# ed-fish/data-efficient-video-transformers

Hardware: AMD Instinct MI355X
Metric: clips/sec fwd+bwd, B=8 T=32 3x224x224 bf16 (higher is better)
Workload: dtype bf16; 1 GPU; ViViT metric shape (SURVEY 8 'M'; BASELINE configs[2]/[3] transformer): B=8/GPU, T=32, 3x224x224, patch 16, d=512, ...; global_batch=8, parallelism=dp1

## Files before the change

### data-efficient-video-transformers_amd/csrc/attention.hip

```cpp
#include "common.h"
#include <cstdlib>

namespace {

__device__ __forceinline__ void wave_lds_sync() {
  asm volatile("s_waitcnt lgkmcnt(0)" ::: "memory");
  __builtin_amdgcn_wave_barrier();
}

constexpr float kLog2e = 1.4426950408889634f;
constexpr float kLn2 = 0.6931471805599453f;

struct AttnParams {
  const void *q, *k, *v, *o, *d_o;
  void *out, *dq, *dk, *dv;
  float* lse;
  float* delta;
  int B, H, Lq, Lk, dh;
  int64_t q_sb, q_sh, q_sl, k_sb, k_sh, k_sl, v_sb, v_sh, v_sl, o_sb, o_sh, o_sl;
  float scale;
  int Lkp;
  int Lqp;
  int patch_off;
  uint32_t drop_thr;
// ... 963 lines not shown
__global__ __launch_bounds__(1024) void attn_bwd_dkv_mfma_kernel(const AttnParams p) {
  extern __shared__ __attribute__((aligned(16))) char smem[];
  using V8 = typename Elem16<E>::v8;
  const int lane = threadIdx.x & 63, wid = threadIdx.x >> 6, W = blockDim.x >> 6;
  const int g = lane >> 4, li = lane & 15;
  const int b = blockIdx.x / p.H, h = blockIdx.x % p.H;
  const E* qb = (const E*)p.q + b * p.q_sb + h * p.q_sh;
  const E* kb = (const E*)p.k + b * p.k_sb + h * p.k_sh;
  const E* vb = (const E*)p.v + b * p.v_sb + h * p.v_sh;
  const E* gb = (const E*)p.d_o + b * p.o_sb + h * p.o_sh;
  E* dkb = (E*)p.dk + b * p.k_sb + h * p.k_sh;
  E* dvb = (E*)p.dv + b * p.v_sb + h * p.v_sh;
  const float* lse = p.lse + ((int64_t)b * p.H + h) * p.Lq;
  const float* delta = p.delta + ((int64_t)b * p.H + h) * p.Lq;
  char* qs = smem;
  char* gs = smem + p.Lqp * kRowBytes;
  float* l2s = reinterpret_cast<float*>(smem + 2 * p.Lqp * kRowBytes);
  float* dls = l2s + p.Lqp;
  const int nkt = (p.Lk + 15) >> 4, nqp = NQP ? NQP : p.Lqp >> 5;
  auto load_rows = [&](int kt, V8* kf, V8* vf) {
    const int kj = kt * 16 + li;
    const int krow = kj < p.Lk ? kj : p.Lk - 1;
#pragma unroll
    for (int kk = 0; kk < 2; ++kk) {
      kf[kk] = *reinterpret_cast<const V8*>(kb + (int64_t)krow * p.k_sl + kk * 32 + g * 8);
      vf[kk] = *reinterpret_cast<const V8*>(vb + (int64_t)krow * p.v_sl + kk * 32 + g * 8);
    }
  };
  V8 kf[2], vf[2];
  load_rows(wid, kf, vf);
  const int sr = (int)threadIdx.x < p.Lq ? (int)threadIdx.x : p.Lq - 1;
  const float lse0 = lse[sr], dl0 = delta[sr];
  stage_images<E>(qs, qb, p.q_sl, gs, gb, p.o_sl, p.Lq, p.Lqp);
  if ((int)threadIdx.x < p.Lqp) {
    l2s[threadIdx.x] = (int)threadIdx.x < p.Lq ? -lse0 * kLog2e : 0.f;
    dls[threadIdx.x] = (int)threadIdx.x < p.Lq ? -dl0 : 0.f;
  }
  for (int r = threadIdx.x + blockDim.x; r < p.Lqp; r += blockDim.x) {
    l2s[r] = r < p.Lq ? -lse[r] * kLog2e : 0.f;
    dls[r] = r < p.Lq ? -delta[r] : 0.f;
  }
  __syncthreads();

  const float c2 = p.scale * kLog2e;
  char* patch = p.patch_off >= 0 ? smem + p.patch_off + wid * 2048 : nullptr;
  for (int kt = wid; kt < nkt; kt += W) {
    asm volatile("" ::: "memory");
    f32x4 dk[4], dv[4];
#pragma unroll
    for (int dt = 0; dt < 4; ++dt) {
      dk[dt] = f32x4{0.f, 0.f, 0.f, 0.f};
      dv[dt] = f32x4{0.f, 0.f, 0.f, 0.f};
    }
    const f32x2 c2v = {c2, c2};
    auto step = [&](int qp) {
      f32x4 s[2], dp[2];
#pragma unroll
      for (int tt = 0; tt < 2; ++tt) {
        s[tt] = f32x4{0.f, 0.f, 0.f, 0.f};
        dp[tt] = f32x4{0.f, 0.f, 0.f, 0.f};
#pragma unroll
        for (int kk = 0; kk < 2; ++kk) {
          s[tt] = Elem16<E>::mma(img_row_frag<E>(qs, (2 * qp + tt) * 16, kk, g, li), kf[kk], s[tt]);
          dp[tt] = Elem16<E>::mma(img_row_frag<E>(gs, (2 * qp + tt) * 16, kk, g, li), vf[kk], dp[tt]);
        }
      }
#pragma unroll
      for (int tt = 0; tt < 2; ++tt) {
        const int q0 = (2 * qp + tt) * 16 + 4 * g;
        const f32x4 l2 = *reinterpret_cast<const f32x4*>(l2s + q0);
        const f32x4 dl = *reinterpret_cast<const f32x4*>(dls + q0);
#pragma unroll
        for (int r = 0; r < 4; r += 2) {
          const f32x2 x = __builtin_elementwise_fma(f32x2{s[tt][r], s[tt][r + 1]}, c2v, f32x2{l2[r], l2[r + 1]});
          const f32x2 d = f32x2{dp[tt][r], dp[tt][r + 1]} + f32x2{dl[r], dl[r + 1]};
          const f32x2 pr = {__builtin_amdgcn_exp2f(x[0]), __builtin_amdgcn_exp2f(x[1])};
          const f32x2 ds = pr * d;
          s[tt][r] = pr[0];
          s[tt][r + 1] = pr[1];
          dp[tt][r] = ds[0];
          dp[tt][r + 1] = ds[1];
        }
      }
      const V8 pf = pack_pair<E>(s[0], s[1]);
      const V8 dsf = pack_pair<E>(dp[0], dp[1]);
#pragma unroll
      for (int dt = 0; dt < 4; ++dt) {
        dv[dt] = Elem16<E>::mma(img_tr_frag<E>(gs, 2 * qp, 2 * qp + 1, dt * 16, g, li), pf, dv[dt]);
        dk[dt] = Elem16<E>::mma(img_tr_frag<E>(qs, 2 * qp, 2 * qp + 1, dt * 16, g, li), dsf, dk[dt]);
      }
    };
    if constexpr (NQP > 0) {
#pragma unroll
      for (int qp = 0; qp < NQP; ++qp) step(qp);
    } else {
      for (int qp = 0; qp < nqp; ++qp) step(qp);
    }
    if (kt + W < nkt) load_rows(kt + W, kf, vf);
    store_tile<E>(patch, dkb, p.k_sl, kt * 16, p.Lk, dk, p.scale, lane);
    store_tile<E>(patch, dvb, p.v_sl, kt * 16, p.Lk, dv, 1.0f, lane);
  }
}

constexpr int kStripRow = 80;

template <typename E>
__device__ __forceinline__ typename Elem16<E>::v8 strip_tr_frag(const char* strip, int ta, int tb, int col0, int g, int li) {
  const int qq = li >> 2, pp = li & 3;
  typename Elem16<E>::v4 half[2];
#pragma unroll
  for (int hf = 0; hf < 2; ++hf) {
    const int r = 16 * (hf ? tb : ta) + 4 * g + qq;
    half[hf] = Elem16<E>::tr_read(strip + r * kStripRow + col0 * 2 + 8 * pp);
  }
  return __builtin_shufflevector(half[0], half[1], 0, 1, 2, 3, 4, 5, 6, 7);
}

template <typename E, int NCH>
__device__ __forceinline__ void stage_bwd_operands(char* qs, const E* q, int64_t q_sl, char* gs, const E* g, const E* o, int64_t o_sl,
                                                   char* ks, const E* k, int64_t k_sl, int Lq, int Lk, int rows_pad, float* dls) {
  using V8 = typename Elem16<E>::v8;
  const int total = rows_pad * 8, nt = blockDim.x;
  V8 vq[NCH], vg[NCH], vo[NCH], vk[NCH];
#pragma unroll
  for (int u = 0; u < NCH; ++u) {
    const int idx = min((int)threadIdx.x + u * nt, total - 1);
    const int r = idx >> 3, c = idx & 7;
    const int rq = r < Lq ? r : 0, rk = r < Lk ? r : 0;
    vq[u] = *reinterpret_cast<const V8*>(q + (int64_t)rq * q_sl + c * 8);
    vg[u] = *reinterpret_cast<const V8*>(g + (int64_t)rq * o_sl + c * 8);
    vo[u] = *reinterpret_cast<const V8*>(o + (int64_t)rq * o_sl + c * 8);
    vk[u] = *reinterpret_cast<const V8*>(k + (int64_t)rk * k_sl + c * 8);
  }
  __builtin_amdgcn_sched_barrier(0);
  const V8 zero = {0, 0, 0, 0, 0, 0, 0, 0};
#pragma unroll
  for (int u = 0; u < NCH; ++u) {
    const int idx = min((int)threadIdx.x + u * nt, total - 1);
    const int r = idx >> 3, off = img_off(r, idx & 7);
    const bool lq = r < Lq, lk = r < Lk;
    *reinterpret_cast<V8*>(qs + off) = lq ? vq[u] : zero;
    *reinterpret_cast<V8*>(gs + off) = lq ? vg[u] : zero;
    *reinterpret_cast<V8*>(ks + off) = lk ? vk[u] : zero;
    float d = 0.f;
#pragma unroll
    for (int j = 0; j < 8; ++j) d = fmaf((float)vg[u][j], (float)vo[u][j], d);
    d += __shfl_xor(d, 1, 64);
    d += __shfl_xor(d, 2, 64);
    d += __shfl_xor(d, 4, 64);
    if ((idx & 7) == 0) dls[r] = lq ? -d : 0.f;
  }
}

template <typename E, int NP>
__global__ __launch_bounds__(512) void attn_bwd_fused_kernel(const AttnParams p) {
  extern __shared__ __attribute__((aligned(16))) char smem[];
  using V8 = typename Elem16<E>::v8;
  using V4 = typename Elem16<E>::v4;
  constexpr int LP = 32 * NP;
  const int lane = threadIdx.x & 63;
  const int wid = __builtin_amdgcn_readfirstlane(threadIdx.x >> 6);
  const int W = blockDim.x >> 6, WC = W - 1;
  const int g = lane >> 4, li = lane & 15;
  const int b = blockIdx.x / p.H, h = blockIdx.x % p.H;
  const E* qb = (const E*)p.q + b * p.q_sb + h * p.q_sh;
  const E* kb = (const E*)p.k + b * p.k_sb + h * p.k_sh;
  const E* vb = (const E*)p.v + b * p.v_sb + h * p.v_sh;
  const E* ob = (const E*)p.o + b * p.o_sb + h * p.o_sh;
  const E* gb = (const E*)p.d_o + b * p.o_sb + h * p.o_sh;
  E* dqb = (E*)p.dq + b * p.q_sb + h * p.q_sh;
  E* dkb = (E*)p.dk + b * p.k_sb + h * p.k_sh;
  E* dvb = (E*)p.dv + b * p.v_sb + h * p.v_sh;
  const float* lse = p.lse + ((int64_t)b * p.H + h) * p.Lq;
  char* qs = smem;
  char* gs = qs + LP * kRowBytes;
  char* ks = gs + LP * kRowBytes;
  char* strip0 = ks + LP * kRowBytes;
  float* l2s = reinterpret_cast<float*>(strip0 + 2 * LP * kStripRow);
  float* dls = l2s + LP;
  char* patch = reinterpret_cast<char*>(dls + LP) + wid * 2048;

  V8 kf[2][2], vf[2][2];
  if (wid < WC) {
#pragma unroll
    for (int j = 0; j < 2; ++j) {
      const int kj = (2 * wid + j) * 16 + li;
      const int krow = kj < p.Lk ? kj : p.Lk - 1;
#pragma unroll
      for (int kk = 0; kk < 2; ++kk) {
        kf[j][kk] = *reinterpret_cast<const V8*>(kb + (int64_t)krow * p.k_sl + kk * 32 + g * 8);
        vf[j][kk] = *reinterpret_cast<const V8*>(vb + (int64_t)krow * p.v_sl + kk * 32 + g * 8);
      }
    }
  }
  {
    const int r = threadIdx.x;
    const float l = lse[r < p.Lq ? r : 0];
    stage_bwd_operands<E, 4>(qs, qb, p.q_sl, gs, gb, ob, p.o_sl, ks, kb, p.k_sl, p.Lq, p.Lk, LP, dls);
    if (r < LP) l2s[r] = r < p.Lq ? -l * kLog2e : 0.f;
  }
  __syncthreads();
  const float c2 = p.scale * kLog2e;
  if (wid < WC) {
    f32x4 dk[2][4], dv[2][4];
#pragma unroll
    for (int j = 0; j < 2; ++j)
#pragma unroll
      for (int dt = 0; dt < 4; ++dt) {
        dk[j][dt] = f32x4{0.f, 0.f, 0.f, 0.f};
        dv[j][dt] = f32x4{0.f, 0.f, 0.f, 0.f};
      }
    const f32x2 c2v = {c2, c2};
    const bool kvalid[2] = {(2 * wid) * 16 + li < p.Lk, (2 * wid + 1) * 16 + li < p.Lk};
    char* myrow[2] = {strip0 + ((2 * wid) * 16 + li) * kStripRow + g * 8, strip0 + ((2 * wid + 1) * 16 + li) * kStripRow + g * 8};
#pragma unroll
    for (int qp = 0; qp < NP; ++qp) {
      asm volatile("" ::: "memory");
      V8 qfr[2][2], gfr[2][2];
#pragma unroll
      for (int tt = 0; tt < 2; ++tt)
#pragma unroll
        for (int kk = 0; kk < 2; ++kk) {
          qfr[tt][kk] = img_row_frag<E>(qs, (2 * qp + tt) * 16, kk, g, li);
          gfr[tt][kk] = img_row_frag<E>(gs, (2 * qp + tt) * 16, kk, g, li);
        }
      f32x4 l2[2], dl[2];
#pragma unroll
      for (int tt = 0; tt < 2; ++tt) {
        l2[tt] = *reinterpret_cast<const f32x4*>(l2s + (2 * qp + tt) * 16 + 4 * g);
        dl[tt] = *reinterpret_cast<const f32x4*>(dls + (2 * qp + tt) * 16 + 4 * g);
      }
      V8 pf[2], dsf[2];
#pragma unroll
      for (int j = 0; j < 2; ++j) {
        f32x4 s[2], dp[2];
#pragma unroll
        for (int tt = 0; tt < 2; ++tt) {
          s[tt] = f32x4{0.f, 0.f, 0.f, 0.f};
          dp[tt] = f32x4{0.f, 0.f, 0.f, 0.f};
#pragma unroll
          for (int kk = 0; kk < 2; ++kk) {
            s[tt] = Elem16<E>::mma(qfr[tt][kk], kf[j][kk], s[tt]);
            dp[tt] = Elem16<E>::mma(gfr[tt][kk], vf[j][kk], dp[tt]);
          }
        }
#pragma unroll
        for (int tt = 0; tt < 2; ++tt)
#pragma unroll
          for (int r = 0; r < 4; r += 2) {
            const f32x2 x = __builtin_elementwise_fma(f32x2{s[tt][r], s[tt][r + 1]}, c2v, f32x2{l2[tt][r], l2[tt][r + 1]});
            const f32x2 d = f32x2{dp[tt][r], dp[tt][r + 1]} + f32x2{dl[tt][r], dl[tt][r + 1]};
            f32x2 pr = {__builtin_amdgcn_exp2f(x[0]), __builtin_amdgcn_exp2f(x[1])};
            if (!kvalid[j]) pr = f32x2{0.f, 0.f};
            const f32x2 ds = pr * d;
            s[tt][r] = pr[0];
            s[tt][r + 1] = pr[1];
            dp[tt][r] = ds[0];
            dp[tt][r + 1] = ds[1];
          }
        pf[j] = pack_pair<E>(s[0], s[1]);
        dsf[j] = pack_pair<E>(dp[0], dp[1]);
      }
#pragma unroll
      for (int j = 0; j < 2; ++j) {
        char* row = myrow[j] + (qp & 1) * (LP * kStripRow);
        *reinterpret_cast<V4*>(row) = __builtin_shufflevector(dsf[j], dsf[j], 0, 1, 2, 3);
        *reinterpret_cast<V4*>(row + 32) = __builtin_shufflevector(dsf[j], dsf[j], 4, 5, 6, 7);
      }
#pragma unroll
      for (int dt = 0; dt < 4; ++dt) {
        const V8 gt = img_tr_frag<E>(gs, 2 * qp, 2 * qp + 1, dt * 16, g, li);
        const V8 qt = img_tr_frag<E>(qs, 2 * qp, 2 * qp + 1, dt * 16, g, li);
#pragma unroll
        for (int j = 0; j < 2; ++j) {
          dv[j][dt] = Elem16<E>::mma(gt, pf[j], dv[j][dt]);
          dk[j][dt] = Elem16<E>::mma(qt, dsf[j], dk[j][dt]);
        }
      }
      __syncthreads();
    }
#pragma unroll
    for (int j = 0; j < 2; ++j) {
      const int k0 = (2 * wid + j) * 16;
      if (k0 < p.Lk) {
        store_tile<E>(patch, dkb, p.k_sl, k0, p.Lk, dk[j], p.scale, lane);
        store_tile<E>(patch, dvb, p.v_sl, k0, p.Lk, dv[j], 1.0f, lane);
      }
    }
  } else {
    V8 ka[NP][4];
#pragma unroll
    for (int kp = 0; kp < NP; ++kp)
#pragma unroll
      for (int dt = 0; dt < 4; ++dt) ka[kp][dt] = img_tr_frag<E>(ks, 2 * kp, 2 * kp + 1, dt * 16, g, li);
#pragma unroll 1
    for (int qp = 0; qp < NP; ++qp) {
      __syncthreads();
      const char* strip = strip0 + (qp & 1) * (LP * kStripRow);
      V8 bq[NP][2];
#pragma unroll
      for (int kp = 0; kp < NP; ++kp) {
        bq[kp][0] = strip_tr_frag<E>(strip, 2 * kp, 2 * kp + 1, 0, g, li);
        bq[kp][1] = strip_tr_frag<E>(strip, 2 * kp, 2 * kp + 1, 16, g, li);
      }
      f32x4 acc[2][4];
#pragma unroll
      for (int tt = 0; tt < 2; ++tt)
#pragma unroll
        for (int dt = 0; dt < 4; ++dt) acc[tt][dt] = f32x4{0.f, 0.f, 0.f, 0.f};
#pragma unroll
      for (int kp = 0; kp < NP; ++kp)
#pragma unroll
        for (int dt = 0; dt < 4; ++dt) {
          acc[0][dt] = Elem16<E>::mma(ka[kp][dt], bq[kp][0], acc[0][dt]);
          acc[1][dt] = Elem16<E>::mma(ka[kp][dt], bq[kp][1], acc[1][dt]);
        }
#pragma unroll
      for (int tt = 0; tt < 2; ++tt)
        if ((2 * qp + tt) * 16 < p.Lq) store_tile<E>(nullptr, dqb, p.q_sl, (2 * qp + tt) * 16, p.Lq, acc[tt], p.scale, lane);
    }
  }
}

constexpr int kMaxLds = 160 * 1024;

int fill_params(const dvt_attn_desc* d, AttnParams& p, bool bwd, const char* name) {
  DVT_REQUIRE(d, "%s: null descriptor", name);
  DVT_REQUIRE(d->q && d->k && d->v && d->o && d->lse, "%s: null q/k/v/o/lse", name);
  DVT_REQUIRE(d->B >= 0 && d->H > 0 && d->Lq > 0 && d->Lk > 0 && d->dh > 0, "%s: bad sizes", name);
  DVT_REQUIRE(d->B * d->H < (1ll << 31) && d->Lq < (1 << 24) && d->Lk < (1 << 24), "%s: sizes too large", name);
  if (bwd) DVT_REQUIRE(d->d_o && d->dq && d->dk && d->dv, "%s: null gradient pointer", name);
  p.q = d->q; p.k = d->k; p.v = d->v; p.o = d->o; p.out = d->o; p.d_o = d->d_o;
  p.dq = d->dq; p.dk = d->dk; p.dv = d->dv; p.lse = d->lse; p.delta = nullptr;
  p.B = (int)d->B; p.H = (int)d->H; p.Lq = (int)d->Lq; p.Lk = (int)d->Lk; p.dh = (int)d->dh;
  p.q_sb = d->q_sb; p.q_sh = d->q_sh; p.q_sl = d->q_sl;
  p.k_sb = d->k_sb; p.k_sh = d->k_sh; p.k_sl = d->k_sl;
  p.v_sb = d->v_sb; p.v_sh = d->v_sh; p.v_sl = d->v_sl;
  p.o_sb = d->o_sb; p.o_sh = d->o_sh; p.o_sl = d->o_sl;
  p.scale = d->scale;
  DVT_REQUIRE(d->dropout_p >= 0.f && d->dropout_p < 1.f, "%s: dropout_p must be in [0, 1)", name);
  DVT_REQUIRE(d->dropout_p == 0.f || d->rng_state, "%s: dropout needs rng_state", name);
  p.drop_thr = 0u; p.drop_scale = 1.f; p.rng = d->rng_state; p.rng_off = d->rng_offset;
  if (d->dropout_p > 0.f) {
    const double th = (double)d->dropout_p * 4294967296.0;
    p.drop_thr = th >= 4294967295.0 ? 0xFFFFFFFFu : (uint32_t)(th + 0.5);
    if (p.drop_thr == 0u) p.drop_thr = 1u;
    p.drop_scale = 1.0f / (1.0f - d->dropout_p);
  }
  p.Lkp = (p.Lk + 31) & ~31;
  p.Lqp = (p.Lq + 31) & ~31;
  p.patch_off = -1;

  return DVT_OK;
}

bool strides_vec_ok(const dvt_attn_desc* d) {
  const int64_t s[] = {d->q_sb, d->q_sh, d->q_sl, d->k_sb, d->k_sh, d->k_sl,
                       d->v_sb, d->v_sh, d->v_sl, d->o_sb, d->o_sh, d->o_sl};
  for (int64_t x : s)
    if (x % 8) return false;
  return true;
}

bool mfma_fwd_ok(const dvt_attn_desc* d, const AttnParams& p) {
  return d->dropout_p == 0.f && d->scale > 0.f && dvt_is_16bit(d->dtype) && d->dh == DH && strides_vec_ok(d) && dvt_aligned16(d->q) &&
         dvt_aligned16(d->k) && dvt_aligned16(d->v) && dvt_aligned16(d->o) &&
         2 * p.Lkp * kRowBytes <= kMaxLds;
}

bool q1_ok(const dvt_attn_desc* d, const AttnParams& p) {
  return p.Lq == 1 && d->dropout_p == 0.f && dvt_is_16bit(d->dtype) && d->dh == DH && strides_vec_ok(d) &&
         dvt_aligned16(d->q) && dvt_aligned16(d->k) && dvt_aligned16(d->v) && dvt_aligned16(d->o) &&
         (size_t)4 * p.Lkp * sizeof(float) <= (size_t)kMaxLds;
}

bool mfma_bwd_ok(const dvt_attn_desc* d, const AttnParams& p) {
  return mfma_fwd_ok(d, p) && dvt_aligned16(d->d_o) && dvt_aligned16(d->dq) && dvt_aligned16(d->dk) &&
         dvt_aligned16(d->dv) && 2 * p.Lqp * kRowBytes + 2 * p.Lqp * 4 <= kMaxLds;
}

bool fused_bwd_ok(const AttnParams& p) { return p.Lqp == p.Lkp && p.Lkp <= 224; }
size_t fused_bwd_lds(int NP, int waves) {
  const size_t LP = 32 * (size_t)NP;
  return 3 * LP * kRowBytes + 2 * LP * kStripRow + 2 * LP * sizeof(float) + (size_t)waves * 2048;
}

int pick_waves(int tiles, size_t lds_bytes, int cap = 16) {
  int maxw = lds_bytes > 80 * 1024 ? 16 : 8;
  if (maxw > cap) maxw = cap;
  const int rounds = (tiles + maxw - 1) / maxw;
  int w = (tiles + rounds - 1) / rounds;
  return w < 1 ? 1 : w;
}

size_t with_patches(size_t lds, int waves, AttnParams& p) {
  const size_t tot = lds + (size_t)waves * 2048;
  const bool ok = lds <= 80 * 1024 ? 2 * tot <= (size_t)kMaxLds : tot <= (size_t)kMaxLds;
  p.patch_off = ok ? (int)lds : -1;
  return ok ? tot : lds;
}

template <typename K>
int set_lds(K kernel, size_t bytes) {
  if (bytes > 64 * 1024) {
    const hipError_t e = hipFuncSetAttribute((const void*)kernel, hipFuncAttributeMaxDynamicSharedMemorySize, (int)bytes);
    if (e != hipSuccess) return dvt_fail_hip(e, "hipFuncSetAttribute(MaxDynamicSharedMemorySize)");
  }
  return 0;
}

int resolve_fwd(const dvt_attn_desc* d, AttnParams& p, dvt_attn_plan_info& r) {
  r = dvt_attn_plan_info{};
  r.patch = r.patch2 = -1;
  int rc = fill_params(d, p, false, "dvt_attention_fwd");
  if (rc) return rc;
  if (p.B == 0) return DVT_OK;
  if (q1_ok(d, p)) {
    r.family = DVT_ATTN_F_Q1; r.waves = 4; r.lds = (int64_t)4 * p.Lkp * sizeof(float);
    return DVT_OK;
  }
  if (mfma_fwd_ok(d, p)) {
    const size_t lds_img = (size_t)2 * p.Lkp * kRowBytes;
    const int nkp = p.Lkp >> 5;
    r.waves = pick_waves((p.Lq + 15) / 16, lds_img, nkp > 7 && nkp <= 11 ? 12 : 16);
    r.lds = (int64_t)with_patches(lds_img, r.waves, p);
    r.patch = p.patch_off >= 0;
    r.family = nkp <= 11 ? DVT_ATTN_F_RES : DVT_ATTN_F_ONLINE;
    r.count = nkp <= 11 ? nkp : 0;
    return DVT_OK;
  }
  const int nt_s = p.Lq * p.dh >= 4096 ? 512 : 256;
  const size_t lds_s = ((size_t)(p.Lq + 2 * p.Lk) * small_dhp(p.dh) +
                        (size_t)small_parts(p.Lq, p.Lk, nt_s) * p.Lq * small_lp(p.Lk)) * sizeof(float);
  if (d->dtype != DVT_F32 && d->dtype != DVT_BF16 && d->dtype != DVT_F16)
    DVT_UNSUPPORTED("dvt_attention_fwd: dtype %d not supported", d->dtype);
  if (p.Lq <= kSmallL && p.Lk <= kSmallL && p.dh <= kSmallDh && lds_s <= (size_t)kMaxLds) {
    r.family = DVT_ATTN_F_SMALL; r.waves = nt_s / 64; r.lds = (int64_t)lds_s;
    return DVT_OK;
  }
  const size_t lds = (size_t)4 * (p.dh + p.Lk) * sizeof(float);
  if (lds > (size_t)kMaxLds) DVT_UNSUPPORTED("dvt_attention_fwd: Lk = %d, dh = %d exceed the LDS budget", p.Lk, p.dh);
  r.family = DVT_ATTN_F_GENERIC; r.waves = 4; r.lds = (int64_t)lds;
  return DVT_OK;
}

int resolve_bwd(const dvt_attn_desc* d, AttnParams& p, AttnParams& pq, AttnParams& pkv, dvt_attn_plan_info& r) {
  r = dvt_attn_plan_info{};
  r.patch = r.patch2 = -1;
  int rc = fill_params(d, p, true, "dvt_attention_bwd");
  if (rc) return rc;
  pq = pkv = p;
  if (p.B == 0) return DVT_OK;
  if (q1_ok(d, p) && dvt_aligned16(d->d_o) && dvt_aligned16(d->dq) && dvt_aligned16(d->dk) && dvt_aligned16(d->dv)) {
    r.family = DVT_ATTN_B_Q1; r.waves = 4;
    return DVT_OK;
  }
  if (mfma_bwd_ok(d, p) && fused_bwd_ok(p) && !d->bwd_two_pass) {
    const int NP = p.Lkp >> 5;
    r.family = DVT_ATTN_B_FUSED; r.count = NP;
    r.waves = NP + 1;
    r.lds = (int64_t)fused_bwd_lds(NP, r.waves);
    return DVT_OK;
  }
  if (mfma_bwd_ok(d, p)) {
    const size_t img_q = (size_t)2 * p.Lkp * kRowBytes;
    const size_t img_kv = (size_t)2 * p.Lqp * kRowBytes + (size_t)2 * p.Lqp * sizeof(float);
    r.family = DVT_ATTN_B_PAIR; r.workspace = 1;
    r.count = (p.Lkp >> 5) <= 11 ? p.Lkp >> 5 : 0;
    r.count2 = (p.Lqp >> 5) <= 11 ? p.Lqp >> 5 : 0;
    r.waves = pick_waves((p.Lq + 15) / 16, img_q);
    r.waves2 = pick_waves((p.Lk + 15) / 16, img_kv);
    r.lds = (int64_t)with_patches(img_q, r.waves, pq);
    r.lds2 = (int64_t)with_patches(img_kv, r.waves2, pkv);
    r.patch = pq.patch_off >= 0; r.patch2 = pkv.patch_off >= 0;
    return DVT_OK;
  }
  if (d->dtype != DVT_F32 && d->dtype != DVT_BF16 && d->dtype != DVT_F16)
    DVT_UNSUPPORTED("dvt_attention_bwd: dtype %d not supported", d->dtype);
  const int nt_s = p.Lq * p.dh >= 4096 ? 512 : 256;
  const size_t lds_s = ((size_t)2 * (p.Lq + p.Lk) * small_dhp(p.dh) +
                        (size_t)2 * small_parts(p.Lq, p.Lk, nt_s) * p.Lq * small_lp(p.Lk) +
                        (size_t)2 * p.Lk * small_lp(p.Lq)) * sizeof(float);
  if (p.Lq <= kSmallL && p.Lk <= kSmallL && p.dh <= kSmallDh && lds_s <= (size_t)kMaxLds) {
    r.family = DVT_ATTN_B_SMALL; r.waves = nt_s / 64; r.lds = (int64_t)lds_s;
    return DVT_OK;
  }
  const size_t lds_q = (size_t)4 * (2 * p.dh + p.Lk) * sizeof(float);
  const size_t lds_kv = (size_t)4 * (2 * p.dh + 2 * p.Lq) * sizeof(float);
  if (lds_q > (size_t)kMaxLds || lds_kv > (size_t)kMaxLds)
    DVT_UNSUPPORTED("dvt_attention_bwd: Lq = %d, Lk = %d, dh = %d exceed the LDS budget", p.Lq, p.Lk, p.dh);
  r.family = DVT_ATTN_B_GENERIC; r.workspace = 1; r.waves = r.waves2 = 4;
  r.lds = (int64_t)lds_q; r.lds2 = (int64_t)lds_kv;
  return DVT_OK;
}

}

extern "C" {

size_t dvt_attention_bwd_workspace_bytes(const dvt_attn_desc* d) {
  if (!d) return 0;
  return (size_t)d->B * (size_t)d->H * (size_t)d->Lq * sizeof(float);
}

int dvt_attention_plan(const dvt_attn_desc* d, int bwd, dvt_attn_plan_info* info) {
  DVT_REQUIRE(info, "dvt_attention_plan: null info");
  AttnParams p, pq, pkv;
  return bwd ? resolve_bwd(d, p, pq, pkv, *info) : resolve_fwd(d, p, *info);
}

int dvt_attention_fwd(const dvt_attn_desc* d, dvt_stream_t stream) {
  AttnParams p;
  dvt_attn_plan_info r;
  int rc = resolve_fwd(d, p, r);
  if (rc) return rc;
  if (p.B == 0) return DVT_OK;
  hipStream_t st = (hipStream_t)stream;
  const size_t lds = (size_t)r.lds;
  if (r.family == DVT_ATTN_F_Q1) {
    const dim3 grid((unsigned)dvt_cdiv((int64_t)p.B * p.H, 4)), block(256);
    DVT_DISPATCH_16BIT(d->dtype, E, {
      if (int rc_ = set_lds(attn_fwd_q1_kernel<E>, lds)) return rc_;
      hipLaunchKernelGGL((attn_fwd_q1_kernel<E>), grid, block, lds, st, p);
    });
    DVT_LAUNCH_CHECK("dvt_attention_fwd(q1)");
    return DVT_OK;
  }
  if (r.family == DVT_ATTN_F_RES || r.family == DVT_ATTN_F_ONLINE) {
    const dim3 grid((unsigned)(p.B * p.H)), block(64 * r.waves);
#define DVT_ATTN_FWD_RES(NKP)                                                               \
  case NKP:                                                                                 \
    if (int rc_ = set_lds(attn_fwd_mfma_res_kernel<E, NKP>, lds)) return rc_;                                         \
    hipLaunchKernelGGL((attn_fwd_mfma_res_kernel<E, NKP>), grid, block, lds, st, p);        \
    break
    DVT_DISPATCH_16BIT(d->dtype, E, {
      switch (r.count) {
        DVT_ATTN_FWD_RES(1); DVT_ATTN_FWD_RES(2); DVT_ATTN_FWD_RES(3); DVT_ATTN_FWD_RES(4);
        DVT_ATTN_FWD_RES(5); DVT_ATTN_FWD_RES(6); DVT_ATTN_FWD_RES(7); DVT_ATTN_FWD_RES(8);
        DVT_ATTN_FWD_RES(9); DVT_ATTN_FWD_RES(10); DVT_ATTN_FWD_RES(11);
        default:
          if (int rc_ = set_lds(attn_fwd_mfma_kernel<E>, lds)) return rc_;
          hipLaunchKernelGGL((attn_fwd_mfma_kernel<E>), grid, block, lds, st, p);
      }
    });
#undef DVT_ATTN_FWD_RES
    DVT_LAUNCH_CHECK("dvt_attention_fwd(mfma)");
    return DVT_OK;
  }
  if (r.family == DVT_ATTN_F_SMALL) {
    const dim3 grid((unsigned)(p.B * p.H)), block(64 * r.waves);
#define DVT_ATTN_SMALL_FWD(T)                                                   \
  do {                                                                          \
    if (int rc_ = set_lds(attn_small_fwd_kernel<T>, lds)) return rc_;                                   \
    hipLaunchKernelGGL((attn_small_fwd_kernel<T>), grid, block, lds, st, p);  \
  } while (0)
    if (d->dtype == DVT_F32) DVT_ATTN_SMALL_FWD(float);
    else if (d->dtype == DVT_BF16) DVT_ATTN_SMALL_FWD(bf16);
    else DVT_ATTN_SMALL_FWD(f16);
#undef DVT_ATTN_SMALL_FWD
    DVT_LAUNCH_CHECK("dvt_attention_fwd(short)");
    return DVT_OK;
  }
  const int64_t rows = (int64_t)p.B * p.H * p.Lq;
  const dim3 grid((unsigned)dvt_cdiv(rows, 4)), block(256);
  if (d->dtype == DVT_F32) {
    if (int rc_ = set_lds(attn_fwd_generic_kernel<float>, lds)) return rc_;
    hipLaunchKernelGGL((attn_fwd_generic_kernel<float>), grid, block, lds, st, p);
  } else if (d->dtype == DVT_BF16) {
    if (int rc_ = set_lds(attn_fwd_generic_kernel<bf16>, lds)) return rc_;
    hipLaunchKernelGGL((attn_fwd_generic_kernel<bf16>), grid, block, lds, st, p);
  } else {
    if (int rc_ = set_lds(attn_fwd_generic_kernel<f16>, lds)) return rc_;
    hipLaunchKernelGGL((attn_fwd_generic_kernel<f16>), grid, block, lds, st, p);
  }
  DVT_LAUNCH_CHECK("dvt_attention_fwd(generic)");
  return DVT_OK;
}

int dvt_attention_bwd(const dvt_attn_desc* d, dvt_stream_t stream) {
  AttnParams p, pq, pkv;
  dvt_attn_plan_info r;
  int rc = resolve_bwd(d, p, pq, pkv, r);
  if (rc) return rc;
  if (p.B == 0) return DVT_OK;
  hipStream_t st = (hipStream_t)stream;
  if (r.family == DVT_ATTN_B_Q1) {
    const dim3 grid((unsigned)dvt_cdiv((int64_t)p.B * p.H, 4)), block(256);
    DVT_DISPATCH_16BIT(d->dtype, E, hipLaunchKernelGGL((attn_bwd_q1_kernel<E>), grid, block, 0, st, p));
    DVT_LAUNCH_CHECK("dvt_attention_bwd(q1)");
    return DVT_OK;
  }
  if (r.family == DVT_ATTN_B_FUSED) {
    const size_t lds = (size_t)r.lds;
    const dim3 grid((unsigned)(p.B * p.H)), block(64 * r.waves);
#define DVT_ATTN_BWD_FUSED(N)                                                               \
  case N:                                                                                   \
    if (int rc_ = set_lds(attn_bwd_fused_kernel<E, N>, lds)) return rc_;                                              \
    hipLaunchKernelGGL((attn_bwd_fused_kernel<E, N>), grid, block, lds, st, p);             \
    break
    DVT_DISPATCH_16BIT(d->dtype, E, {
      switch (r.count) {
        DVT_ATTN_BWD_FUSED(1); DVT_ATTN_BWD_FUSED(2); DVT_ATTN_BWD_FUSED(3); DVT_ATTN_BWD_FUSED(4);
        DVT_ATTN_BWD_FUSED(5); DVT_ATTN_BWD_FUSED(6); DVT_ATTN_BWD_FUSED(7);
      }
    });
#undef DVT_ATTN_BWD_FUSED
    DVT_LAUNCH_CHECK("dvt_attention_bwd(fused)");
    return DVT_OK;
  }
  if (r.family == DVT_ATTN_B_PAIR) {
    DVT_REQUIRE(d->workspace, "dvt_attention_bwd: workspace (dvt_attention_bwd_workspace_bytes) required");
    pq.delta = pkv.delta = (float*)d->workspace;
    const dim3 grid((unsigned)(p.B * p.H));
    const dim3 block_q(64 * r.waves), block_kv(64 * r.waves2);
    const size_t lds_q = (size_t)r.lds, lds_kv = (size_t)r.lds2;
#define DVT_ATTN_BWD_DQ(NKP)                                                                \
  case NKP:                                                                                 \
    if (int rc_ = set_lds(attn_bwd_dq_mfma_kernel<E, NKP>, lds_q)) return rc_;                                        \
    hipLaunchKernelGGL((attn_bwd_dq_mfma_kernel<E, NKP>), grid, block_q, lds_q, st, pq);     \
    break
#define DVT_ATTN_BWD_DKV(NQP)                                                               \
  case NQP:                                                                                 \
    if (int rc_ = set_lds(attn_bwd_dkv_mfma_kernel<E, NQP>, lds_kv)) return rc_;                                      \
    hipLaunchKernelGGL((attn_bwd_dkv_mfma_kernel<E, NQP>), grid, block_kv, lds_kv, st, pkv);  \
    break
    DVT_DISPATCH_16BIT(d->dtype, E, {
      switch (r.count) {
        DVT_ATTN_BWD_DQ(1); DVT_ATTN_BWD_DQ(2); DVT_ATTN_BWD_DQ(3); DVT_ATTN_BWD_DQ(4);
        DVT_ATTN_BWD_DQ(5); DVT_ATTN_BWD_DQ(6); DVT_ATTN_BWD_DQ(7); DVT_ATTN_BWD_DQ(8);
        DVT_ATTN_BWD_DQ(9); DVT_ATTN_BWD_DQ(10); DVT_ATTN_BWD_DQ(11);
        default:
          if (int rc_ = set_lds(attn_bwd_dq_mfma_kernel<E, 0>, lds_q)) return rc_;
          hipLaunchKernelGGL((attn_bwd_dq_mfma_kernel<E, 0>), grid, block_q, lds_q, st, pq);
      }
      switch (r.count2) {
        DVT_ATTN_BWD_DKV(1); DVT_ATTN_BWD_DKV(2); DVT_ATTN_BWD_DKV(3); DVT_ATTN_BWD_DKV(4);
        DVT_ATTN_BWD_DKV(5); DVT_ATTN_BWD_DKV(6); DVT_ATTN_BWD_DKV(7); DVT_ATTN_BWD_DKV(8);
        DVT_ATTN_BWD_DKV(9); DVT_ATTN_BWD_DKV(10); DVT_ATTN_BWD_DKV(11);
        default:
          if (int rc_ = set_lds(attn_bwd_dkv_mfma_kernel<E, 0>, lds_kv)) return rc_;
          hipLaunchKernelGGL((attn_bwd_dkv_mfma_kernel<E, 0>), grid, block_kv, lds_kv, st, pkv);
      }
    });
#undef DVT_ATTN_BWD_DQ
#undef DVT_ATTN_BWD_DKV
    DVT_LAUNCH_CHECK("dvt_attention_bwd(dkdv)");
    return DVT_OK;
  }
  if (r.family == DVT_ATTN_B_SMALL) {
    const size_t lds_s = (size_t)r.lds;
    const dim3 grid((unsigned)(p.B * p.H)), block(64 * r.waves);
#define DVT_ATTN_SMALL_BWD(T)                                                   \
  do {                                                                          \
    if (int rc_ = set_lds(attn_small_bwd_kernel<T>, lds_s)) return rc_;                                   \
    hipLaunchKernelGGL((attn_small_bwd_kernel<T>), grid, block, lds_s, st, p);  \
  } while (0)
    if (d->dtype == DVT_F32) DVT_ATTN_SMALL_BWD(float);
    else if (d->dtype == DVT_BF16) DVT_ATTN_SMALL_BWD(bf16);
    else DVT_ATTN_SMALL_BWD(f16);
#undef DVT_ATTN_SMALL_BWD
    DVT_LAUNCH_CHECK("dvt_attention_bwd(short)");
    return DVT_OK;
  }
  DVT_REQUIRE(d->workspace, "dvt_attention_bwd: workspace (dvt_attention_bwd_workspace_bytes) required");
  p.delta = (float*)d->workspace;
  const size_t lds_q = (size_t)r.lds, lds_kv = (size_t)r.lds2;
  const int64_t qrows = (int64_t)p.B * p.H * p.Lq, krows = (int64_t)p.B * p.H * p.Lk;
  const dim3 block(256);
#define DVT_ATTN_BWD_GENERIC(T)                                                                   \
  do {                                                                                            \
    if (int rc_ = set_lds(attn_bwd_dq_generic_kernel<T>, lds_q)) return rc_;                                                \
    if (int rc_ = set_lds(attn_bwd_dkv_generic_kernel<T>, lds_kv)) return rc_;                                              \
    hipLaunchKernelGGL((attn_delta_kernel<T>), dim3((unsigned)dvt_cdiv(qrows, 4)), block, 0, st, p); \
    hipLaunchKernelGGL((attn_bwd_dq_generic_kernel<T>), dim3((unsigned)dvt_cdiv(qrows, 4)), block, lds_q, st, p); \
    hipLaunchKernelGGL((attn_bwd_dkv_generic_kernel<T>), dim3((unsigned)dvt_cdiv(krows, 4)), block, lds_kv, st, p); \
  } while (0)
  if (d->dtype == DVT_F32) DVT_ATTN_BWD_GENERIC(float);
  else if (d->dtype == DVT_BF16) DVT_ATTN_BWD_GENERIC(bf16);
  else DVT_ATTN_BWD_GENERIC(f16);
#undef DVT_ATTN_BWD_GENERIC
  DVT_LAUNCH_CHECK("dvt_attention_bwd(generic)");
  return DVT_OK;
}

}
```

Measured before the change: 1441 clips/s.

## Make fused attention backward persistent with async prefetch of next head's operands

The fused backward kernel now launches at most one block per CU. Each block loops over a contiguous range of (batch, head) items instead of handling one item per block. While computing the current item, the compute waves issue asynchronous LDS DMA loads of the next item's Q, dO and K rows, and prefetch its O, LSE, K and V fragments into registers. The aim is to hide the global-load and staging latency that each block previously paid up front. The cost is extra barriers, more register pressure, and a risk of load imbalance or LDS hazards when the next item's Q/dO/K overwrite buffers still in use.

```diff
diff --git a/data-efficient-video-transformers_amd/csrc/attention.hip b/data-efficient-video-transformers_amd/csrc/attention.hip
--- a/data-efficient-video-transformers_amd/csrc/attention.hip
+++ b/data-efficient-video-transformers_amd/csrc/attention.hip
@@ -1139,6 +1139,40 @@
   }
 }
 
+__device__ __attribute__((aligned(16))) unsigned int attn_zero16[4] = {0u, 0u, 0u, 0u};
+
+template <typename E>
+__device__ __forceinline__ void dma_img_unit(char* img, const E* src, int64_t sl, int L, int unit, int lane) {
+  asm volatile("" : "+s"(unit));
+  const int r = unit * 8 + (lane >> 3), slot = lane & 7;
+  const int c = (((slot >> 1) ^ ((r >> 1) & 3)) << 1) | (slot & 1);
+  const void* s = r < L ? static_cast<const void*>(src + (int64_t)r * sl + c * 8) : static_cast<const void*>(attn_zero16);
+  dvt_dma16(s, img + unit * 1024);
+}
+
+template <typename E>
+struct BwdItem {
+  const E *q, *k, *v, *o, *g;
+  E *dq, *dk, *dv;
+  const float* lse;
+};
+
+template <typename E>
+__device__ __forceinline__ BwdItem<E> bwd_item(const AttnParams& p, int it) {
+  const int b = it / p.H, h = it % p.H;
+  BwdItem<E> x;
+  x.q = (const E*)p.q + b * p.q_sb + h * p.q_sh;
+  x.k = (const E*)p.k + b * p.k_sb + h * p.k_sh;
+  x.v = (const E*)p.v + b * p.v_sb + h * p.v_sh;
+  x.o = (const E*)p.o + b * p.o_sb + h * p.o_sh;
+  x.g = (const E*)p.d_o + b * p.o_sb + h * p.o_sh;
+  x.dq = (E*)p.dq + b * p.q_sb + h * p.q_sh;
+  x.dk = (E*)p.dk + b * p.k_sb + h * p.k_sh;
+  x.dv = (E*)p.dv + b * p.v_sb + h * p.v_sh;
+  x.lse = p.lse + ((int64_t)b * p.H + h) * p.Lq;
+  return x;
+}
+
 template <typename E, int NP>
 __global__ __launch_bounds__(512) void attn_bwd_fused_kernel(const AttnParams p) {
   extern __shared__ __attribute__((aligned(16))) char smem[];
@@ -1149,16 +1183,8 @@
   const int wid = __builtin_amdgcn_readfirstlane(threadIdx.x >> 6);
   const int W = blockDim.x >> 6, WC = W - 1;
   const int g = lane >> 4, li = lane & 15;
-  const int b = blockIdx.x / p.H, h = blockIdx.x % p.H;
-  const E* qb = (const E*)p.q + b * p.q_sb + h * p.q_sh;
-  const E* kb = (const E*)p.k + b * p.k_sb + h * p.k_sh;
-  const E* vb = (const E*)p.v + b * p.v_sb + h * p.v_sh;
-  const E* ob = (const E*)p.o + b * p.o_sb + h * p.o_sh;
-  const E* gb = (const E*)p.d_o + b * p.o_sb + h * p.o_sh;
-  E* dqb = (E*)p.dq + b * p.q_sb + h * p.q_sh;
-  E* dkb = (E*)p.dk + b * p.k_sb + h * p.k_sh;
-  E* dvb = (E*)p.dv + b * p.v_sb + h * p.v_sh;
-  const float* lse = p.lse + ((int64_t)b * p.H + h) * p.Lq;
+  const int n = p.B * p.H;
+  const int it0 = (int)((int64_t)blockIdx.x * n / gridDim.x), it1 = (int)((int64_t)(blockIdx.x + 1) * n / gridDim.x);
   char* qs = smem;
   char* gs = qs + LP * kRowBytes;
   char* ks = gs + LP * kRowBytes;
@@ -1167,6 +1193,7 @@
   float* dls = l2s + LP;
   char* patch = reinterpret_cast<char*>(dls + LP) + wid * 2048;
 
+  BwdItem<E> cur = bwd_item<E>(p, it0);
   V8 kf[2][2], vf[2][2];
   if (wid < WC) {
 #pragma unroll
@@ -1175,136 +1202,209 @@
       const int krow = kj < p.Lk ? kj : p.Lk - 1;
 #pragma unroll
       for (int kk = 0; kk < 2; ++kk) {
-        kf[j][kk] = *reinterpret_cast<const V8*>(kb + (int64_t)krow * p.k_sl + kk * 32 + g * 8);
-        vf[j][kk] = *reinterpret_cast<const V8*>(vb + (int64_t)krow * p.v_sl + kk * 32 + g * 8);
+        kf[j][kk] = *reinterpret_cast<const V8*>(cur.k + (int64_t)krow * p.k_sl + kk * 32 + g * 8);
+        vf[j][kk] = *reinterpret_cast<const V8*>(cur.v + (int64_t)krow * p.v_sl + kk * 32 + g * 8);
       }
     }
   }
   {
     const int r = threadIdx.x;
-    const float l = lse[r < p.Lq ? r : 0];
-    stage_bwd_operands<E, 4>(qs, qb, p.q_sl, gs, gb, ob, p.o_sl, ks, kb, p.k_sl, p.Lq, p.Lk, LP, dls);
+    const float l = cur.lse[r < p.Lq ? r : 0];
+    stage_bwd_operands<E, 4>(qs, cur.q, p.q_sl, gs, cur.g, cur.o, p.o_sl, ks, cur.k, p.k_sl, p.Lq, p.Lk, LP, dls);
     if (r < LP) l2s[r] = r < p.Lq ? -l * kLog2e : 0.f;
   }
-  __syncthreads();
   const float c2 = p.scale * kLog2e;
   if (wid < WC) {
-    f32x4 dk[2][4], dv[2][4];
-#pragma unroll
-    for (int j = 0; j < 2; ++j)
-#pragma unroll
-      for (int dt = 0; dt < 4; ++dt) {
-        dk[j][dt] = f32x4{0.f, 0.f, 0.f, 0.f};
-        dv[j][dt] = f32x4{0.f, 0.f, 0.f, 0.f};
-      }
-    const f32x2 c2v = {c2, c2};
-    const bool kvalid[2] = {(2 * wid) * 16 + li < p.Lk, (2 * wid + 1) * 16 + li < p.Lk};
-    char* myrow[2] = {strip0 + ((2 * wid) * 16 + li) * kStripRow + g * 8, strip0 + ((2 * wid + 1) * 16 + li) * kStripRow + g * 8};
-#pragma unroll
-    for (int qp = 0; qp < NP; ++qp) {
-      asm volatile("" ::: "memory");
-      V8 qfr[2][2], gfr[2][2];
-#pragma unroll
-      for (int tt = 0; tt < 2; ++tt)
-#pragma unroll
-        for (int kk = 0; kk < 2; ++kk) {
-          qfr[tt][kk] = img_row_frag<E>(qs, (2 * qp + tt) * 16, kk, g, li);
-          gfr[tt][kk] = img_row_frag<E>(gs, (2 * qp + tt) * 16, kk, g, li);
+    V8 no[4];
+    float nl = 0.f;
+    for (int it = it0; it < it1; ++it) {
+      const bool more = it + 1 < it1;
+      const BwdItem<E> nxt = bwd_item<E>(p, more ? it + 1 : it);
+      __syncthreads();
+      int lane = threadIdx.x & 63;
+      asm volatile("" : "+v"(lane));
+      const int g = lane >> 4, li = lane & 15;
+      const int tc = wid * 64 + lane;
+      if (it > it0) {
+#pragma unroll
+        for (int u = 0; u < 4; ++u) {
+          const int idx = tc + u * 64 * WC, r = idx >> 3;
+          const V8 vg = *reinterpret_cast<const V8*>(gs + img_off(r, idx & 7));
+          float d = 0.f;
+#pragma unroll
+          for (int j = 0; j < 8; ++j) d = fmaf((float)vg[j], (float)no[u][j], d);
+          d += __shfl_xor(d, 1, 64);
+          d += __shfl_xor(d, 2, 64);
+          d += __shfl_xor(d, 4, 64);
+          if ((idx & 7) == 0) dls[r] = r < p.Lq ? -d : 0.f;
         }
-      f32x4 l2[2], dl[2];
-#pragma unroll
-      for (int tt = 0; tt < 2; ++tt) {
-        l2[tt] = *reinterpret_cast<const f32x4*>(l2s + (2 * qp + tt) * 16 + 4 * g);
-        dl[tt] = *reinterpret_cast<const f32x4*>(dls + (2 * qp + tt) * 16 + 4 * g);
-      }
-      V8 pf[2], dsf[2];
-#pragma unroll
-      for (int j = 0; j < 2; ++j) {
-        f32x4 s[2], dp[2];
+        if (tc < LP) l2s[tc] = tc < p.Lq ? -nl * kLog2e : 0.f;
+      }
+      __syncthreads();
+      auto next_rows = [&](int s, int half) {
+#pragma unroll
+        for (int j = 0; j < 12; ++j)
+          if ((j >= NP) == (half == 1) && j % NP == wid) {
+            const int unit = 4 * s + (j & 3);
+            if (j < 4) {
+              if (unit * 8 < p.Lq) dma_img_unit<E>(qs, nxt.q, p.q_sl, p.Lq, unit, lane);
+            } else if (j < 8) {
+              if (unit * 8 < p.Lq) dma_img_unit<E>(gs, nxt.g, p.o_sl, p.Lq, unit, lane);
+            } else {
+              if (unit * 8 < p.Lk) dma_img_unit<E>(ks, nxt.k, p.k_sl, p.Lk, unit, lane);
+            }
+          }
+      };
+      f32x4 dk[2][4], dv[2][4];
+#pragma unroll
+      for (int j = 0; j < 2; ++j)
+#pragma unroll
+        for (int dt = 0; dt < 4; ++dt) {
+          dk[j][dt] = f32x4{0.f, 0.f, 0.f, 0.f};
+          dv[j][dt] = f32x4{0.f, 0.f, 0.f, 0.f};
+        }
+      const f32x2 c2v = {c2, c2};
+      const bool kvalid[2] = {(2 * wid) * 16 + li < p.Lk, (2 * wid + 1) * 16 + li < p.Lk};
+      char* myrow[2] = {strip0 + ((2 * wid) * 16 + li) * kStripRow + g * 8, strip0 + ((2 * wid + 1) * 16 + li) * kStripRow + g * 8};
+#pragma unroll
+      for (int qp = 0; qp < NP; ++qp) {
+        if (more && qp > 0) next_rows(qp - 1, 0);
+        asm volatile("" ::: "memory");
+        V8 qfr[2][2], gfr[2][2];
+#pragma unroll
+        for (int tt = 0; tt < 2; ++tt)
+#pragma unroll
+          for (int kk = 0; kk < 2; ++kk) {
+            qfr[tt][kk] = img_row_frag<E>(qs, (2 * qp + tt) * 16, kk, g, li);
+            gfr[tt][kk] = img_row_frag<E>(gs, (2 * qp + tt) * 16, kk, g, li);
+          }
+        f32x4 l2[2], dl[2];
 #pragma unroll
         for (int tt = 0; tt < 2; ++tt) {
-          s[tt] = f32x4{0.f, 0.f, 0.f, 0.f};
-          dp[tt] = f32x4{0.f, 0.f, 0.f, 0.f};
-#pragma unroll
-          for (int kk = 0; kk < 2; ++kk) {
-            s[tt] = Elem16<E>::mma(qfr[tt][kk], kf[j][kk], s[tt]);
-            dp[tt] = Elem16<E>::mma(gfr[tt][kk], vf[j][kk], dp[tt]);
+          l2[tt] = *reinterpret_cast<const f32x4*>(l2s + (2 * qp + tt) * 16 + 4 * g);
+          dl[tt] = *reinterpret_cast<const f32x4*>(dls + (2 * qp + tt) * 16 + 4 * g);
+        }
+        V8 pf[2], dsf[2];
+#pragma unroll
+        for (int j = 0; j < 2; ++j) {
+          f32x4 s[2], dp[2];
+#pragma unroll
+          for (int tt = 0; tt < 2; ++tt) {
+            s[tt] = f32x4{0.f, 0.f, 0.f, 0.f};
+            dp[tt] = f32x4{0.f, 0.f, 0.f, 0.f};
+#pragma unroll
+            for (int kk = 0; kk < 2; ++kk) {
+              s[tt] = Elem16<E>::mma(qfr[tt][kk], kf[j][kk], s[tt]);
+              dp[tt] = Elem16<E>::mma(gfr[tt][kk], vf[j][kk], dp[tt]);
+            }
+          }
+#pragma unroll
+          for (int tt = 0; tt < 2; ++tt)
+#pragma unroll
+            for (int r = 0; r < 4; r += 2) {
+              const f32x2 x = __builtin_elementwise_fma(f32x2{s[tt][r], s[tt][r + 1]}, c2v, f32x2{l2[tt][r], l2[tt][r + 1]});
+              const f32x2 d = f32x2{dp[tt][r], dp[tt][r + 1]} + f32x2{dl[tt][r], dl[tt][r + 1]};
+              f32x2 pr = {__builtin_amdgcn_exp2f(x[0]), __builtin_amdgcn_exp2f(x[1])};
+              if (!kvalid[j]) pr = f32x2{0.f, 0.f};
+              const f32x2 ds = pr * d;
+              s[tt][r] = pr[0];
+              s[tt][r + 1] = pr[1];
+              dp[tt][r] = ds[0];
+              dp[tt][r + 1] = ds[1];
+            }
+          pf[j] = pack_pair<E>(s[0], s[1]);
+          dsf[j] = pack_pair<E>(dp[0], dp[1]);
+        }
+        if (more && qp > 0) next_rows(qp - 1, 1);
+#pragma unroll
+        for (int j = 0; j < 2; ++j) {
+          char* row = myrow[j] + (qp & 1) * (LP * kStripRow);
+          *reinterpret_cast<V4*>(row) = __builtin_shufflevector(dsf[j], dsf[j], 0, 1, 2, 3);
+          *reinterpret_cast<V4*>(row + 32) = __builtin_shufflevector(dsf[j], dsf[j], 4, 5, 6, 7);
+        }
+#pragma unroll
+        for (int dt = 0; dt < 4; ++dt) {
+          const V8 gt = img_tr_frag<E>(gs, 2 * qp, 2 * qp + 1, dt * 16, g, li);
+          const V8 qt = img_tr_frag<E>(qs, 2 * qp, 2 * qp + 1, dt * 16, g, li);
+#pragma unroll
+          for (int j = 0; j < 2; ++j) {
+            dv[j][dt] = Elem16<E>::mma(gt, pf[j], dv[j][dt]);
+            dk[j][dt] = Elem16<E>::mma(qt, dsf[j], dk[j][dt]);
           }
         }
+        __syncthreads();
+      }
+      if (more) {
+        next_rows(NP - 1, 0);
+        next_rows(NP - 1, 1);
+#pragma unroll
+        for (int u = 0; u < 4; ++u) {
+          const int idx = tc + u * 64 * WC, r = idx >> 3;
+          no[u] = *reinterpret_cast<const V8*>(nxt.o + (int64_t)(r < p.Lq ? r : 0) * p.o_sl + (idx & 7) * 8);
+        }
+        nl = nxt.lse[tc < p.Lq ? tc : 0];
+#pragma unroll
+        for (int j = 0; j < 2; ++j) {
+          const int kj = (2 * wid + j) * 16 + li;
+          const int krow = kj < p.Lk ? kj : p.Lk - 1;
+#pragma unroll
+          for (int kk = 0; kk < 2; ++kk) {
+            kf[j][kk] = *reinterpret_cast<const V8*>(nxt.k + (int64_t)krow * p.k_sl + kk * 32 + g * 8);
+            vf[j][kk] = *reinterpret_cast<const V8*>(nxt.v + (int64_t)krow * p.v_sl + kk * 32 + g * 8);
+          }
+        }
+      }
+#pragma unroll
+      for (int j = 0; j < 2; ++j) {
+        const int k0 = (2 * wid + j) * 16;
+        if (k0 < p.Lk) {
+          store_tile<E>(patch, cur.dk, p.k_sl, k0, p.Lk, dk[j], p.scale, lane);
+          store_tile<E>(patch, cur.dv, p.v_sl, k0, p.Lk, dv[j], 1.0f, lane);
+        }
+      }
+      if (more) asm volatile("s_waitcnt vmcnt(0)" ::: "memory");
+      cur = nxt;
+    }
+  } else {
+    for (int it = it0; it < it1; ++it) {
+      __syncthreads();
+      __syncthreads();
+      int lane = threadIdx.x & 63;
+      asm volatile("" : "+v"(lane));
+      const int g = lane >> 4, li = lane & 15;
+      V8 ka[NP][4];
+#pragma unroll
+      for (int kp = 0; kp < NP; ++kp)
+#pragma unroll
+        for (int dt = 0; dt < 4; ++dt) ka[kp][dt] = img_tr_frag<E>(ks, 2 * kp, 2 * kp + 1, dt * 16, g, li);
+      asm volatile("s_waitcnt lgkmcnt(0)" ::: "memory");
+#pragma unroll 1
+      for (int qp = 0; qp < NP; ++qp) {
+        __syncthreads();
+        const char* strip = strip0 + (qp & 1) * (LP * kStripRow);
+        V8 bq[NP][2];
+#pragma unroll
+        for (int kp = 0; kp < NP; ++kp) {
+          bq[kp][0] = strip_tr_frag<E>(strip, 2 * kp, 2 * kp + 1, 0, g, li);
+          bq[kp][1] = strip_tr_frag<E>(strip, 2 * kp, 2 * kp + 1, 16, g, li);
+        }
+        f32x4 acc[2][4];
 #pragma unroll
         for (int tt = 0; tt < 2; ++tt)
 #pragma unroll
-          for (int r = 0; r < 4; r += 2) {
-            const f32x2 x = __builtin_elementwise_fma(f32x2{s[tt][r], s[tt][r + 1]}, c2v, f32x2{l2[tt][r], l2[tt][r + 1]});
-            const f32x2 d = f32x2{dp[tt][r], dp[tt][r + 1]} + f32x2{dl[tt][r], dl[tt][r + 1]};
-            f32x2 pr = {__builtin_amdgcn_exp2f(x[0]), __builtin_amdgcn_exp2f(x[1])};
-            if (!kvalid[j]) pr = f32x2{0.f, 0.f};
-            const f32x2 ds = pr * d;
-            s[tt][r] = pr[0];
-            s[tt][r + 1] = pr[1];
-            dp[tt][r] = ds[0];
-            dp[tt][r + 1] = ds[1];
+          for (int dt = 0; dt < 4; ++dt) acc[tt][dt] = f32x4{0.f, 0.f, 0.f, 0.f};
+#pragma unroll
+        for (int kp = 0; kp < NP; ++kp)
+#pragma unroll
+          for (int dt = 0; dt < 4; ++dt) {
+            acc[0][dt] = Elem16<E>::mma(ka[kp][dt], bq[kp][0], acc[0][dt]);
+            acc[1][dt] = Elem16<E>::mma(ka[kp][dt], bq[kp][1], acc[1][dt]);
           }
-        pf[j] = pack_pair<E>(s[0], s[1]);
-        dsf[j] = pack_pair<E>(dp[0], dp[1]);
-      }
-#pragma unroll
-      for (int j = 0; j < 2; ++j) {
-        char* row = myrow[j] + (qp & 1) * (LP * kStripRow);
-        *reinterpret_cast<V4*>(row) = __builtin_shufflevector(dsf[j], dsf[j], 0, 1, 2, 3);
-        *reinterpret_cast<V4*>(row + 32) = __builtin_shufflevector(dsf[j], dsf[j], 4, 5, 6, 7);
-      }
-#pragma unroll
-      for (int dt = 0; dt < 4; ++dt) {
-        const V8 gt = img_tr_frag<E>(gs, 2 * qp, 2 * qp + 1, dt * 16, g, li);
-        const V8 qt = img_tr_frag<E>(qs, 2 * qp, 2 * qp + 1, dt * 16, g, li);
-#pragma unroll
-        for (int j = 0; j < 2; ++j) {
-          dv[j][dt] = Elem16<E>::mma(gt, pf[j], dv[j][dt]);
-          dk[j][dt] = Elem16<E>::mma(qt, dsf[j], dk[j][dt]);
-        }
-      }
-      __syncthreads();
-    }
-#pragma unroll
-    for (int j = 0; j < 2; ++j) {
-      const int k0 = (2 * wid + j) * 16;
-      if (k0 < p.Lk) {
-        store_tile<E>(patch, dkb, p.k_sl, k0, p.Lk, dk[j], p.scale, lane);
-        store_tile<E>(patch, dvb, p.v_sl, k0, p.Lk, dv[j], 1.0f, lane);
-      }
-    }
-  } else {
-    V8 ka[NP][4];
-#pragma unroll
-    for (int kp = 0; kp < NP; ++kp)
-#pragma unroll
-      for (int dt = 0; dt < 4; ++dt) ka[kp][dt] = img_tr_frag<E>(ks, 2 * kp, 2 * kp + 1, dt * 16, g, li);
-#pragma unroll 1
-    for (int qp = 0; qp < NP; ++qp) {
-      __syncthreads();
-      const char* strip = strip0 + (qp & 1) * (LP * kStripRow);
-      V8 bq[NP][2];
-#pragma unroll
-      for (int kp = 0; kp < NP; ++kp) {
-        bq[kp][0] = strip_tr_frag<E>(strip, 2 * kp, 2 * kp + 1, 0, g, li);
-        bq[kp][1] = strip_tr_frag<E>(strip, 2 * kp, 2 * kp + 1, 16, g, li);
-      }
-      f32x4 acc[2][4];
-#pragma unroll
-      for (int tt = 0; tt < 2; ++tt)
-#pragma unroll
-        for (int dt = 0; dt < 4; ++dt) acc[tt][dt] = f32x4{0.f, 0.f, 0.f, 0.f};
-#pragma unroll
-      for (int kp = 0; kp < NP; ++kp)
-#pragma unroll
-        for (int dt = 0; dt < 4; ++dt) {
-          acc[0][dt] = Elem16<E>::mma(ka[kp][dt], bq[kp][0], acc[0][dt]);
-          acc[1][dt] = Elem16<E>::mma(ka[kp][dt], bq[kp][1], acc[1][dt]);
-        }
-#pragma unroll
-      for (int tt = 0; tt < 2; ++tt)
-        if ((2 * qp + tt) * 16 < p.Lq) store_tile<E>(nullptr, dqb, p.q_sl, (2 * qp + tt) * 16, p.Lq, acc[tt], p.scale, lane);
+#pragma unroll
+        for (int tt = 0; tt < 2; ++tt)
+          if ((2 * qp + tt) * 16 < p.Lq) store_tile<E>(nullptr, cur.dq, p.q_sl, (2 * qp + tt) * 16, p.Lq, acc[tt], p.scale, lane);
+      }
+      cur = bwd_item<E>(p, it + 1 < it1 ? it + 1 : it);
     }
   }
 }
@@ -1371,6 +1471,10 @@
   const size_t LP = 32 * (size_t)NP;
   return 3 * LP * kRowBytes + 2 * LP * kStripRow + 2 * LP * sizeof(float) + (size_t)waves * 2048;
 }
+unsigned fused_bwd_grid(const AttnParams& p) {
+  const int64_t n = (int64_t)p.B * p.H, cus = dvt_num_cus();
+  return (unsigned)(n < cus ? n : cus);
+}
 
 int pick_waves(int tiles, size_t lds_bytes, int cap = 16) {
   int maxw = lds_bytes > 80 * 1024 ? 16 : 8;
@@ -1579,7 +1683,7 @@
   }
   if (r.family == DVT_ATTN_B_FUSED) {
     const size_t lds = (size_t)r.lds;
-    const dim3 grid((unsigned)(p.B * p.H)), block(64 * r.waves);
+    const dim3 grid(fused_bwd_grid(p)), block(64 * r.waves);
 #define DVT_ATTN_BWD_FUSED(N)                                                               \
   case N:                                                                                   \
     if (int rc_ = set_lds(attn_bwd_fused_kernel<E, N>, lds)) return rc_;                                              \
```

Result: no change. 1448 clips/s, median of 6 (+0.5%).
